# zengxiaofei/HapHiC

Hardware: NVIDIA H100
Metric: hic_pairs_per_sec_matrix_build (higher is better)
Workload: dtype int32 counts / fp32 matrix

## Files before the change

haphic_b200/csrc/hh_gemm.cu:

```cuda
#include "hh_common.cuh"
#include "hh_internal.cuh"
#include "hh_gemm.cuh"
#include <cuda.h>
#include <cuda_fp16.h>
#include <stdlib.h>
#include <algorithm>

__device__ __forceinline__ uint32_t hg_smem_u32(const void* p) { return (uint32_t)__cvta_generic_to_shared(p); }

__device__ __forceinline__ void hg_mbar_init(uint32_t bar, uint32_t count) {
    asm volatile("mbarrier.init.shared::cta.b64 [%0], %1;" ::"r"(bar), "r"(count) : "memory");
}
__device__ __forceinline__ void hg_fence_barrier_init() { asm volatile("fence.mbarrier_init.release.cluster;" ::: "memory"); }
__device__ __forceinline__ void hg_mbar_wait(uint32_t bar, uint32_t parity) {
    uint32_t ok;
    do {
        asm volatile(
            "{\n\t.reg .pred p;\n\t"
            "mbarrier.try_wait.parity.shared::cta.b64 p, [%1], %2;\n\t"
            "selp.u32 %0, 1, 0, p;\n\t}"
            : "=r"(ok)
            : "r"(bar), "r"(parity)
            : "memory");
    } while (!ok);
// ... 17 lines not shown
__device__ __forceinline__ uint64_t hg_make_desc(uint32_t saddr) {
    uint64_t d = 0;
    d |= (uint64_t)((saddr >> 4) & 0x3FFFu);
    d |= (uint64_t)1 << 16;
    d |= (uint64_t)(1024 >> 4) << 32;
    d |= (uint64_t)1 << 62;
    return d;
}

__device__ __forceinline__ void hg_wgmma_fence() { asm volatile("wgmma.fence.sync.aligned;" ::: "memory"); }
__device__ __forceinline__ void hg_wgmma_commit() { asm volatile("wgmma.commit_group.sync.aligned;" ::: "memory"); }
__device__ __forceinline__ void hg_wgmma_wait0() { asm volatile("wgmma.wait_group.sync.aligned 0;" ::: "memory"); }

#define HG_ACC8(i) "+f"(d[i]), "+f"(d[i + 1]), "+f"(d[i + 2]), "+f"(d[i + 3]), "+f"(d[i + 4]), "+f"(d[i + 5]), "+f"(d[i + 6]), "+f"(d[i + 7])
#define HG_WGMMA_BODY(TYPES)                                                                                                      \
    asm volatile(                                                                                                                 \
        "{\n\t.reg .pred p;\n\tsetp.ne.b32 p, %66, 0;\n\t"                                                                         \
        "wgmma.mma_async.sync.aligned.m64n128k16.f32." TYPES " "                                                                  \
        "{%0, %1, %2, %3, %4, %5, %6, %7, %8, %9, %10, %11, %12, %13, %14, %15, "                                                 \
        "%16, %17, %18, %19, %20, %21, %22, %23, %24, %25, %26, %27, %28, %29, %30, %31, "                                        \
        "%32, %33, %34, %35, %36, %37, %38, %39, %40, %41, %42, %43, %44, %45, %46, %47, "                                         \
        "%48, %49, %50, %51, %52, %53, %54, %55, %56, %57, %58, %59, %60, %61, %62, %63}, "                                       \
        "%64, %65, p, 1, 1, 0, 0;\n\t}"                                                                                           \
        : HG_ACC8(0), HG_ACC8(8), HG_ACC8(16), HG_ACC8(24), HG_ACC8(32), HG_ACC8(40), HG_ACC8(48), HG_ACC8(56)                   \
        : "l"(adesc), "l"(bdesc), "r"(accumulate))
template <bool F16>
__device__ __forceinline__ void hg_wgmma(float (&d)[64], uint64_t adesc, uint64_t bdesc, uint32_t accumulate) {
    if (F16) HG_WGMMA_BODY("f16.f16");
    else HG_WGMMA_BODY("bf16.bf16");
}

#define HG_THREADS 384
#define HG_TILE 128
#define HG_PLANE_BYTES 16384
#define HG_MAX_STAGES 4

struct hh_gemm_args {
    const hh_gemm_item* items;
    int n_items;
    int n;
    int na, nb;
    int npass;
    int pa[8], pb[8];
    int chunk_kb;
    int stages;
    float* m1;
    long long ld;
    int col_lo, col_hi;
    const float* inv_s;
    float out_scale;
    int accumulate;
};

template <bool F16>
__global__ void __launch_bounds__(HG_THREADS, 1)
hh_k_syrk(const __grid_constant__ CUtensorMap tmA, const __grid_constant__ CUtensorMap tmB, const hh_gemm_args a) {
    extern __shared__ uint8_t hg_smem_raw[];
    __shared__ __align__(8) uint64_t s_full[HG_MAX_STAGES];
    __shared__ __align__(8) uint64_t s_empty[HG_MAX_STAGES];

    const int wg = threadIdx.x >> 7, lane = threadIdx.x & 31;
    const uint32_t smem_base = (hg_smem_u32(hg_smem_raw) + 1023u) & ~1023u;
    const uint32_t stage_bytes = (uint32_t)(a.na + a.nb) * HG_PLANE_BYTES;
    const int S = a.stages;

    if (threadIdx.x == 0) {
        for (int s = 0; s < S; ++s) {
            hg_mbar_init(hg_smem_u32(&s_full[s]), 1);
            hg_mbar_init(hg_smem_u32(&s_empty[s]), 8);
        }
        hg_fence_barrier_init();
        hg_prefetch_tmap(&tmA);
        hg_prefetch_tmap(&tmB);
    }
    __syncthreads();

    if (wg == 0) {
        if (threadIdx.x == 0) {
            int s = 0;
            uint32_t ph = 0;
            for (int it = blockIdx.x; it < a.n_items; it += gridDim.x) {
                const hh_gemm_item w = a.items[it];
                for (int seg = 0; seg < 2; ++seg) {
                    for (int kb = w.kb_lo[seg]; kb < w.kb_hi[seg]; ++kb) {
                        hg_mbar_wait(hg_smem_u32(&s_empty[s]), ph ^ 1u);
                        const uint32_t bar = hg_smem_u32(&s_full[s]);
                        hg_mbar_expect_tx(bar, stage_bytes);
                        const uint32_t dst = smem_base + (uint32_t)s * stage_bytes;
                        for (int p = 0; p < a.na; ++p) hg_tma_load_3d(dst + (uint32_t)p * HG_PLANE_BYTES, &tmA, bar, kb * 64, w.m0, p);
                        for (int p = 0; p < a.nb; ++p)
                            hg_tma_load_3d(dst + (uint32_t)(a.na + p) * HG_PLANE_BYTES, &tmB, bar, kb * 64, w.n0, p);
                        if (++s == S) {
                            s = 0;
                            ph ^= 1u;
                        }
                    }
                }
            }
        }
        return;
    }

    const int e = wg - 1;
    const int wq = (threadIdx.x >> 5) & 3;
    int s = 0;
    uint32_t ph = 0;
    float acc[64], racc[64];
    for (int it = blockIdx.x; it < a.n_items; it += gridDim.x) {
        const hh_gemm_item w = a.items[it];
        const int total = (w.kb_hi[0] - w.kb_lo[0]) + (w.kb_hi[1] - w.kb_lo[1]);
#pragma unroll
        for (int j = 0; j < 64; ++j) {
            acc[j] = 0.f;
            racc[j] = 0.f;
        }
        int in_chunk = 0;
        for (int t = 0; t < total; ++t) {
            hg_mbar_wait(hg_smem_u32(&s_full[s]), ph);
            const uint32_t st = smem_base + (uint32_t)s * stage_bytes;
            hg_wgmma_fence();
            for (int p = 0; p < a.npass; ++p) {
                const uint64_t ad = hg_make_desc(st + (uint32_t)a.pa[p] * HG_PLANE_BYTES + (uint32_t)e * (64u * 128u));
                const uint64_t bd = hg_make_desc(st + (uint32_t)(a.na + a.pb[p]) * HG_PLANE_BYTES);
#pragma unroll
                for (int k = 0; k < 4; ++k)
                    hg_wgmma<F16>(acc, ad + (uint64_t)(2 * k), bd + (uint64_t)(2 * k), (in_chunk | p | k) ? 1u : 0u);
            }
            hg_wgmma_commit();
            hg_wgmma_wait0();
            __syncwarp();
            if (lane == 0) hg_mbar_arrive(hg_smem_u32(&s_empty[s]));
            if (++s == S) {
                s = 0;
                ph ^= 1u;
            }
            if (++in_chunk == a.chunk_kb || t + 1 == total) {
#pragma unroll
                for (int j = 0; j < 64; ++j) racc[j] = __fadd_rn(racc[j], acc[j]);
                in_chunk = 0;
            }
        }
#pragma unroll
        for (int h = 0; h < 2; ++h) {
            const int r = w.m0 + 64 * e + 16 * wq + (lane >> 2) + 8 * h;
            if (r >= w.m_end) continue;
            if (w.flags & HH_GEMM_DIRECT) {
                float* __restrict__ dst = a.m1 + (ptrdiff_t)(r - w.out_row0);
#pragma unroll
                for (int q = 0; q < 16; ++q) {
#pragma unroll
                    for (int b = 0; b < 2; ++b) {
                        const int c = w.n0 + 8 * q + 2 * (lane & 3) + b;
                        if (c < w.n_end && c >= a.col_lo && c < a.col_hi) {
                            float* __restrict__ o = dst + (size_t)(c - a.col_lo) * (size_t)a.ld;
                            const float x = racc[4 * q + 2 * h + b];
                            const float v = a.inv_s ? x * __ldg(a.inv_s + c) : x * a.out_scale;
                            *o = a.accumulate ? __fadd_rn(*o, v) : v;
                        }
                    }
                }
            }
            if ((w.flags & HH_GEMM_MIRROR) && r >= a.col_lo && r < a.col_hi) {
                const float sr = a.inv_s ? __ldg(a.inv_s + r) : a.out_scale;
                float* __restrict__ dst = a.m1 + (size_t)(r - a.col_lo) * (size_t)a.ld - (ptrdiff_t)w.out_row0;
#pragma unroll
                for (int q = 0; q < 16; ++q) {
                    const int c = w.n0 + 8 * q + 2 * (lane & 3);
                    const float v0 = racc[4 * q + 2 * h] * sr, v1 = racc[4 * q + 2 * h + 1] * sr;
                    if (c + 1 < w.n_end && w.out_row0 == 0) {
                        float2 v = make_float2(v0, v1);
                        if (a.accumulate) {
                            const float2 old = *reinterpret_cast<const float2*>(dst + c);
                            v = make_float2(__fadd_rn(old.x, v.x), __fadd_rn(old.y, v.y));
                        }
                        *reinterpret_cast<float2*>(dst + c) = v;
                    } else {
                        if (c < w.n_end) dst[c] = a.accumulate ? __fadd_rn(dst[c], v0) : v0;
                        if (c + 1 < w.n_end) dst[c + 1] = a.accumulate ? __fadd_rn(dst[c + 1], v1) : v1;
                    }
                }
            }
        }
    }
}

__global__ void hh_k_gemm_colsum(const int64_t* __restrict__ colptr, const float* __restrict__ val, int n, double* __restrict__ s,
                                 float* __restrict__ inv_s, int* __restrict__ flags) {
    const int c = blockIdx.x * (blockDim.x >> 5) + (threadIdx.x >> 5);
    if (c >= n) return;
    const int lane = threadIdx.x & 31;
    double t = 0.0;
    for (int64_t p = colptr[c] + lane; p < colptr[c + 1]; p += 32) t += fabs((double)val[p]);
    t = hh_warp_sum(t);
    if (lane == 0) {
        s[c] = t;
        inv_s[c] = (t != 0.0) ? (float)(1.0 / t) : 1.f;
        if (t >= 8388608.0) atomicOr(flags, 4);
    }
}

__global__ void hh_k_gemm_valstats(const float* __restrict__ val, int64_t nnz, int* __restrict__ flags) {
    int f = 0;
    for (int64_t p = (int64_t)blockIdx.x * blockDim.x + threadIdx.x; p < nnz; p += (int64_t)gridDim.x * blockDim.x) {
        const float v = val[p];
        if (!(v >= 0.f && v < 65536.f && v == floorf(v))) f |= 1;
        if (v > 256.f) f |= 2;
        if (v > 2048.f) f |= 8;
    }
    f = __reduce_or_sync(HH_FULL_MASK, f);
    if ((threadIdx.x & 31) == 0 && f) atomicOr(flags, f);
}

__device__ __forceinline__ void hg_split3(float x, unsigned short& h1, unsigned short& h2, unsigned short& h3) {
    const uint32_t b1 = __float_as_uint(x) & 0xFFFF0000u;
    const float r1 = x - __uint_as_float(b1);
// ... 13 lines not shown
    const int c = blockIdx.x;
    const int64_t p0 = colptr[c], p1 = colptr[c + 1];
    for (int group = 0; group < 2; ++group) {
        const int np = group ? nb : na;
        unsigned short* __restrict__ out = (group ? B : A) + (size_t)c * (size_t)ldk;
        for (long long seg0 = k0; seg0 < k0 + ldk; seg0 += HG_SEG) {
            const int seg_n = (int)((k0 + ldk - seg0 < HG_SEG) ? (k0 + ldk - seg0) : HG_SEG);
            uint4* z = reinterpret_cast<uint4*>(hg_row);
            for (int q = threadIdx.x; q < 3 * HG_SEG / 8; q += blockDim.x) z[q] = make_uint4(0u, 0u, 0u, 0u);
            __syncthreads();
            for (int64_t p = p0 + threadIdx.x; p < p1; p += blockDim.x) {
                const long long k = row[p];
                if (k < seg0 || k >= seg0 + seg_n) continue;
                const float v = fminf(val[p], clip);
                const double sk = s[k];
                unsigned short h1 = 0, h2 = 0, h3 = 0;
                if (!scaled) {
                    float x = v;
                    if (group) x = (sk != 0.0) ? (float)((double)v / sk) : v;
                    hg_split3(x, h1, h2, h3);
                } else {
                    const int e = (sk != 0.0) ? (int)((__double2hiint(sk) >> 20) & 0x7ff) - 1022 : 0;
                    if (!group) {
                        const float xa = v * __int_as_float((127 - e) << 23);
                        h1 = a_f16 ? __half_as_ushort(__float2half_rn(xa)) : (unsigned short)(__float_as_uint(xa) >> 16);
                    } else {
                        const float x = (sk != 0.0) ? (float)((double)v / sk) : v;
                        const float xs = x * __int_as_float((127 + e) << 23);
                        const __half hi = __float2half_rn(xs);
                        const __half lo = __float2half_rn(xs - __half2float(hi));
                        h1 = __half_as_ushort(hi);
                        h2 = __half_as_ushort(lo);
                    }
                }
                const int kk = (int)(k - seg0);
                hg_row[kk] = h1;
                if (np > 1) hg_row[HG_SEG + kk] = h2;
                if (np > 2) hg_row[2 * HG_SEG + kk] = h3;
            }
            __syncthreads();
            for (int pl = 0; pl < np; ++pl) {
                const uint4* src = reinterpret_cast<const uint4*>(hg_row + (size_t)pl * HG_SEG);
                uint4* dst = reinterpret_cast<uint4*>(out + (size_t)pl * (size_t)plane + (size_t)(seg0 - k0));
                for (int q = threadIdx.x; q < seg_n / 8; q += blockDim.x) dst[q] = src[q];
            }
            __syncthreads();
        }
    }
}

typedef CUresult (*hg_encode_fn)(CUtensorMap*, CUtensorMapDataType, cuuint32_t, void*, const cuuint64_t*, const cuuint64_t*, const cuuint32_t*,
                                 const cuuint32_t*, CUtensorMapInterleave, CUtensorMapSwizzle, CUtensorMapL2promotion, CUtensorMapFloatOOBfill);

static int hg_encode(CUtensorMap* tm, void* base, int rows, int kdim, long long ldk, long long plane_elems, int planes, int fmt) {
    static hg_encode_fn fn = nullptr;
    if (!fn) {
        void* p = nullptr;
        cudaDriverEntryPointQueryResult q;
        HH_CUDA(cudaGetDriverEntryPoint("cuTensorMapEncodeTiled", &p, cudaEnableDefault, &q));
        HH_REQUIRE(p != nullptr && q == cudaDriverEntryPointSuccess, HH_ERR_CUDA, "hh_gemm: the driver does not export cuTensorMapEncodeTiled");
        fn = reinterpret_cast<hg_encode_fn>(p);
    }
    const cuuint64_t dims[3] = {(cuuint64_t)kdim, (cuuint64_t)rows, (cuuint64_t)planes};
    const cuuint64_t strides[2] = {(cuuint64_t)ldk * 2ull, (cuuint64_t)plane_elems * 2ull};
    const cuuint32_t box[3] = {64u, 128u, 1u};
    const cuuint32_t estr[3] = {1u, 1u, 1u};
    const CUresult r = fn(tm, fmt == HH_GEMM_F16 ? CU_TENSOR_MAP_DATA_TYPE_FLOAT16 : CU_TENSOR_MAP_DATA_TYPE_BFLOAT16, 3, base, dims, strides, box, estr, CU_TENSOR_MAP_INTERLEAVE_NONE,
                          CU_TENSOR_MAP_SWIZZLE_128B, CU_TENSOR_MAP_L2_PROMOTION_L2_256B, CU_TENSOR_MAP_FLOAT_OOB_FILL_NONE);
    HH_REQUIRE(r == CUDA_SUCCESS, HH_ERR_CUDA, "hh_gemm: cuTensorMapEncodeTiled failed (%d)", (int)r);
    return HH_OK;
}

static int hg_env_int(const char* name, int dflt) {
    const char* v = getenv(name);
    return (v && *v) ? atoi(v) : dflt;
}

template <bool F16>
static int hg_launch(hh_ctx* ctx, const CUtensorMap& tmA, const CUtensorMap& tmB, const hh_gemm_args& a, size_t smem) {
    auto kern = hh_k_syrk<F16>;
    HH_CUDA(cudaFuncSetAttribute(kern, cudaFuncAttributeMaxDynamicSharedMemorySize, (int)smem));
    int grid = ctx->sm_count;
    if (grid > a.n_items) grid = a.n_items;
    if (grid < 1) grid = 1;
    HH_LAUNCH(ctx, kern, grid, HG_THREADS, smem, tmA, tmB, a);
    return HH_OK;
}

int hh_gemm_run(hh_ctx* ctx, const hh_gemm_operand& A, const hh_gemm_operand& B, const hh_gemm_item* d_items, int n_items, int npass,
                const int* pa, const int* pb, int chunk_kb, float* out, long long ld, int col_lo, int col_hi, const float* scale,
                int* stages_out, float out_scale, int accumulate) {
    HH_REQUIRE(n_items >= 1 && npass >= 1 && npass <= 8, HH_ERR_ARG, "hh_gemm_run: bad work list");
    HH_REQUIRE(A.fmt == B.fmt, HH_ERR_ARG, "hh_gemm_run: wgmma takes one 16-bit format for both operands");
    CUtensorMap tmA, tmB;
    HH_CHECK(hg_encode(&tmA, (void*)A.base, A.rows, A.kdim, A.ldk, A.plane, A.planes, A.fmt));
    HH_CHECK(hg_encode(&tmB, (void*)B.base, B.rows, B.kdim, B.ldk, B.plane, B.planes, B.fmt));
    hh_gemm_args a;
    memset(&a, 0, sizeof(a));
    a.items = d_items;
    a.n_items = n_items;
    a.na = A.planes;
    a.nb = B.planes;
    a.npass = npass;
    for (int p = 0; p < npass; ++p) {
        a.pa[p] = pa[p];
        a.pb[p] = pb[p];
    }
    a.chunk_kb = chunk_kb < 1 ? (1 << 30) : chunk_kb;
    const size_t stage_bytes = (size_t)(A.planes + B.planes) * HG_PLANE_BYTES;
    int stages = (int)((ctx->smem_optin - 2048) / stage_bytes);
    if (stages > HG_MAX_STAGES) stages = HG_MAX_STAGES;
    HH_REQUIRE(stages >= 2, HH_ERR_UNSUPPORTED, "hh_gemm: shared memory too small for two pipeline stages");
    a.stages = stages;
    if (stages_out) *stages_out = stages;
    a.m1 = out;
    a.ld = ld;
    a.col_lo = col_lo;
    a.col_hi = col_hi;
    a.inv_s = scale;
    a.out_scale = out_scale;
    a.accumulate = accumulate;
    const size_t smem = (size_t)stages * stage_bytes + 1024;
    return A.fmt == HH_GEMM_F16 ? hg_launch<true>(ctx, tmA, tmB, a, smem) : hg_launch<false>(ctx, tmA, tmB, a, smem);
}

static const int HG_P1[3][2] = {{0, 0}, {0, 1}, {0, 2}};
static const int HG_P3[6][2] = {{0, 0}, {0, 1}, {1, 0}, {0, 2}, {1, 1}, {2, 0}};

int hh_gemm_passes(int na, int* pa, int* pb) {
    const int(*pl)[2] = na == 1 ? HG_P1 : HG_P3;
    const int np = na == 1 ? 3 : 6;
    for (int p = 0; p < np; ++p) {
        pa[p] = pl[p][0];
        pb[p] = pl[p][1];
    }
    return np;
}

void hh_gemm_kchunks(int n, int planes, long long* kw_out, int* kchunks_out) {
    const long long ldk = ((long long)n + 63) & ~63ll;
    const double plane_bytes_all = (double)planes * (double)(ldk * (long long)n) * 2.0;
    int kchunks = (int)(plane_bytes_all / 16.0e9) + 1;
    kchunks = hg_env_int("HH_GEMM_KCHUNKS", kchunks);
    if (kchunks < 1) kchunks = 1;
    const long long kw = ((((long long)n + kchunks - 1) / kchunks) + 63) & ~63ll;
    *kw_out = kw;
    *kchunks_out = (int)(((long long)n + kw - 1) / kw);
}

size_t hh_gemm_preexpand_plane_bytes(int n) {
    size_t most = 0;
    for (int planes : {3, 4, 6}) {
        long long kw = 0;
        int kc = 0;
        hh_gemm_kchunks(n, planes, &kw, &kc);
        const size_t b = (size_t)planes * (size_t)kw * (size_t)n * 2;
        if (b > most) most = b;
    }
    return most;
}

int hh_gemm_preexpand(hh_ctx* ctx, const hh_matrix* m, int col_lo, int col_hi, float* d_m1, long long ld, const hh_gemm_item* h_items,
                      int n_items, hh_gemm_stats* st) {
    const int n = m->n;
    HH_REQUIRE(n >= 1 && n_items >= 1, HH_ERR_ARG, "hh_gemm_preexpand: empty problem");
    double* d_s = nullptr;
    float* d_inv = nullptr;
    int* d_flags = nullptr;
    unsigned short *d_A = nullptr, *d_B = nullptr;
    hh_gemm_item* d_items = nullptr;
    cudaEvent_t ev[3] = {nullptr, nullptr, nullptr};
    int rc = [&]() -> int {
        for (int k = 0; k < 3; ++k) HH_CUDA(cudaEventCreate(&ev[k]));
        HH_CHECK(hh_dmalloc(&d_s, (size_t)n));
        HH_CHECK(hh_dmalloc(&d_inv, (size_t)n));
        HH_CHECK(hh_dmalloc(&d_flags, 1));
        HH_CUDA(cudaEventRecord(ev[0], ctx->stream));
        HH_CUDA(cudaMemsetAsync(d_flags, 0, sizeof(int), ctx->stream));
        HH_LAUNCH(ctx, hh_k_gemm_colsum, (n + 7) / 8, 256, 0, m->d_colptr, m->d_val, n, d_s, d_inv, d_flags);
        HH_LAUNCH(ctx, hh_k_gemm_valstats, ctx->sm_count * 8, 256, 0, m->d_val, m->nnz, d_flags);
        int flags = 0;
        HH_CUDA(cudaMemcpyAsync(&flags, d_flags, sizeof(int), cudaMemcpyDeviceToHost, ctx->stream));
        HH_CUDA(cudaStreamSynchronize(ctx->stream));
        const char* fmt_env = getenv("HH_GEMM_FMT");
        int enc = 2;
        if (fmt_env && !strcmp(fmt_env, "bf16")) enc = 0;
        if (flags & (1 | 4)) enc = 0;
        const int na = (flags & 1) ? 3 : 1;
        const int nb = enc ? 2 : 3;
        const float clip = (flags & 1) ? 3.0e38f : (enc == 2 ? 2048.f : 256.f);
        const int fmt_a = enc == 2 ? HH_GEMM_F16 : HH_GEMM_BF16, fmt_b = enc ? HH_GEMM_F16 : HH_GEMM_BF16;
        long long kw = 0;
        int kchunks = 0;
        hh_gemm_kchunks(n, na + nb, &kw, &kchunks);
        const long long plane_c = kw * (long long)n;
        HH_CHECK(hh_ws_alloc(ctx, &d_A, (size_t)plane_c * (size_t)na));
        HH_CHECK(hh_ws_alloc(ctx, &d_B, (size_t)plane_c * (size_t)nb));
        HH_CUDA(cudaMemsetAsync(d_m1, 0, (size_t)ld * (size_t)(col_hi - col_lo) * sizeof(float), ctx->stream));
        HH_CHECK(hh_dmalloc(&d_items, (size_t)n_items));
        int pa[8], pb[8];
        int npass = hh_gemm_passes(na, pa, pb);
        if (enc) {
            npass = 2;
            pa[0] = pa[1] = 0;
            pb[0] = 0;
            pb[1] = 1;
        }
        const int chunk = hg_env_int("HH_GEMM_CHUNK", npass > 3 ? 1 : (npass == 3 ? 2 : 3));
        int stages = 0;
        float densify_ms = 0.f, gemm_ms = 0.f;
        const float stats_ms = 0.f;
        std::vector<hh_gemm_item> items_c(h_items, h_items + n_items);
        for (int kc = 0; kc < kchunks; ++kc) {
            const long long k0 = (long long)kc * kw;
            const long long k1 = std::min((long long)n, k0 + kw);
            HH_CUDA(cudaEventRecord(ev[0], ctx->stream));
            {
                auto kd = hh_k_gemm_densify;
                const size_t dsm = (size_t)3 * HG_SEG * sizeof(unsigned short);
                HH_CUDA(cudaFuncSetAttribute(kd, cudaFuncAttributeMaxDynamicSharedMemorySize, (int)dsm));
                HH_LAUNCH(ctx, kd, n, 1024, dsm, m->d_colptr, m->d_row, m->d_val, n, d_s, d_A, na, d_B, nb, kw, plane_c, clip, enc ? 1 : 0,
                          enc == 2 ? 1 : 0, k0);
            }
            const int nkb_c = (int)((k1 - k0 + 63) / 64);
            for (auto& w : items_c) {
                w.kb_lo[0] = 0;
                w.kb_hi[0] = nkb_c;
            }
            HH_CUDA(cudaMemcpyAsync(d_items, items_c.data(), (size_t)n_items * sizeof(hh_gemm_item), cudaMemcpyHostToDevice, ctx->stream));
            hh_gemm_operand A = {d_A, na, n, (int)(k1 - k0), kw, plane_c, fmt_a};
            hh_gemm_operand B = {d_B, nb, n, (int)(k1 - k0), kw, plane_c, fmt_b};
            HH_CUDA(cudaEventRecord(ev[1], ctx->stream));
            HH_CHECK(hh_gemm_run(ctx, A, B, d_items, n_items, npass, pa, pb, chunk, d_m1, ld, col_lo, col_hi, d_inv, &stages, 1.0f,
                                 kc > 0 ? 1 : 0));
            HH_CUDA(cudaEventRecord(ev[2], ctx->stream));
            HH_CUDA(cudaStreamSynchronize(ctx->stream));
            float t0 = 0.f, t1 = 0.f;
            HH_CUDA(cudaEventElapsedTime(&t0, ev[0], ev[1]));
            HH_CUDA(cudaEventElapsedTime(&t1, ev[1], ev[2]));
            densify_ms += t0;
            gemm_ms += t1;
        }
        HH_CUDA(cudaEventRecord(ev[2], ctx->stream));
        HH_CUDA(cudaStreamSynchronize(ctx->stream));
        if (st) {
            memset(st, 0, sizeof(*st));
            st->a_planes = na;
            st->clipped = (clip < 1.0e38f && (flags & (clip > 256.f ? 8 : 2))) ? 1 : 0;
            st->clip = clip;
            st->fmt_a = fmt_a;
            st->fmt_b = fmt_b;
            st->b_planes = nb;
            st->passes = npass;
            st->cta_group = 1;
            st->stages = stages;
            st->chunk_kb = chunk < 1 ? (1 << 30) : chunk;
            st->densify_ms = densify_ms + stats_ms;
            st->gemm_ms = gemm_ms;
            st->k_chunks = kchunks;
            double kb = 0.0;
            for (int i = 0; i < n_items; ++i) kb += (double)((h_items[i].kb_hi[0] - h_items[i].kb_lo[0]) + (h_items[i].kb_hi[1] - h_items[i].kb_lo[1]));
            const double tile = (double)HG_TILE;
            st->flops = 2.0 * tile * tile * 64.0 * kb * (double)npass;
        }
        return HH_OK;
    }();
    hh_dfree(d_s);
    hh_dfree(d_inv);
    hh_dfree(d_flags);
    hh_ws_free(ctx, d_A);
    hh_ws_free(ctx, d_B);
    hh_dfree(d_items);
    for (int k = 0; k < 3; ++k)
        if (ev[k]) cudaEventDestroy(ev[k]);
    return rc;
}


#define HG_BLK_SHIFT 14
__global__ void __launch_bounds__(128)
hh_k_blk_densify(const int* __restrict__ len, const uint2* __restrict__ ent, int cap, const int* __restrict__ list, int nlist,
                 const int* __restrict__ comp_lo, const int* __restrict__ comp_hi, unsigned short* __restrict__ Bt, long long ldk,
                 long long plane, int f16) {
    extern __shared__ __align__(16) unsigned short hb_row[];
    const int j = list[blockIdx.x];
    const int lo = comp_lo[j], width = comp_hi[j] - lo;
    uint4* z = reinterpret_cast<uint4*>(hb_row);
    for (int q = threadIdx.x; q < (int)(3 * ldk / 8); q += 128) z[q] = make_uint4(0u, 0u, 0u, 0u);
    __syncthreads();
    const int L = len[j];
    const uint2* __restrict__ e = ent + (size_t)j * (size_t)cap;
    for (int p = threadIdx.x; p < L; p += 128) {
        const uint2 t = e[p];
        const unsigned kk = t.x - (unsigned)lo;
        if (kk < (unsigned)width) {
            unsigned short h1, h2, h3 = 0;
            if (f16) {
                const float xs = ldexpf(__uint_as_float(t.y), HG_BLK_SHIFT);
                const __half hi = __float2half_rn(xs);
                h1 = __half_as_ushort(hi);
                h2 = __half_as_ushort(__float2half_rn(xs - __half2float(hi)));
            } else {
                hg_split3(__uint_as_float(t.y), h1, h2, h3);
            }
            hb_row[kk] = h1;
            hb_row[ldk + kk] = h2;
            hb_row[2 * ldk + kk] = h3;
        }
    }
    __syncthreads();
    for (int pl = 0; pl < (f16 ? 2 : 3); ++pl) {
        const uint4* src = reinterpret_cast<const uint4*>(hb_row + (size_t)pl * (size_t)ldk);
        uint4* dst = reinterpret_cast<uint4*>(Bt + (size_t)pl * (size_t)plane + (size_t)j * (size_t)ldk);
        for (int q = threadIdx.x; q < (int)(ldk / 8); q += 128) dst[q] = src[q];
    }
}

__global__ void __launch_bounds__(256)
hh_k_blk_transpose(const unsigned short* __restrict__ Bt, unsigned short* __restrict__ A, int n, const int* __restrict__ comp_lo,
                   const int* __restrict__ comp_hi, long long ldk, long long plane) {
    __shared__ unsigned short tile[32][34];
    const int r0 = blockIdx.x * 32, kk0 = blockIdx.y * 32;
    const unsigned short* __restrict__ src = Bt + (size_t)blockIdx.z * (size_t)plane;
    unsigned short* __restrict__ dst = A + (size_t)blockIdx.z * (size_t)plane;
    const int tx = threadIdx.x, ty = threadIdx.y;
    const int rl = min(r0 + 31, n - 1);
    const bool same = (r0 + 31 < n) && comp_lo[r0] == comp_lo[rl];
    if (same) {
        const int lo = comp_lo[r0], width = comp_hi[r0] - lo;
        const bool fits = width <= (int)ldk;
        for (int y = ty; y < 32; y += 8) {
            const int kk = kk0 + y;
            tile[y][tx] = (fits && kk < width) ? src[(size_t)(lo + kk) * (size_t)ldk + (size_t)(r0 - lo + tx)] : (unsigned short)0;
        }
        __syncthreads();
        for (int y = ty; y < 32; y += 8) dst[(size_t)(r0 + y) * (size_t)ldk + (size_t)(kk0 + tx)] = tile[tx][y];
    } else {
        for (int y = ty; y < 32; y += 8) {
            const int r = r0 + y;
            if (r >= n) continue;
            const int lo = comp_lo[r], width = comp_hi[r] - lo;
            const int kk = kk0 + tx;
            dst[(size_t)r * (size_t)ldk + (size_t)kk] =
                (width <= (int)ldk && kk < width) ? src[(size_t)(lo + kk) * (size_t)ldk + (size_t)(r - lo)] : (unsigned short)0;
        }
    }
}

float hh_gemm_blk_out_scale(int f16) { return f16 ? ldexpf(1.0f, -2 * HG_BLK_SHIFT) : 1.0f; }

int hh_gemm_blk_operands(hh_ctx* ctx, const int* d_len, const void* d_ent, int cap, const int* d_list, int nlist, const int* d_comp_lo,
                         const int* d_comp_hi, int n, unsigned short* d_A, unsigned short* d_Bt, long long ldk, int f16) {
    const long long plane = ldk * (long long)n;
    auto kd = hh_k_blk_densify;
    const size_t dsm = (size_t)3 * (size_t)ldk * sizeof(unsigned short);
    HH_CUDA(cudaFuncSetAttribute(kd, cudaFuncAttributeMaxDynamicSharedMemorySize, (int)dsm));
    if (nlist > 0)
        HH_LAUNCH(ctx, kd, nlist, 128, dsm, d_len, reinterpret_cast<const uint2*>(d_ent), cap, d_list, nlist, d_comp_lo, d_comp_hi, d_Bt, ldk,
                  plane, f16);
    dim3 grid((unsigned)((n + 31) / 32), (unsigned)(ldk / 32), f16 ? 2u : 3u), block(32, 8);
    hh_k_blk_transpose<<<grid, block, 0, ctx->stream>>>(d_Bt, d_A, n, d_comp_lo, d_comp_hi, ldk, plane);
    ctx->launches++;
    HH_CUDA(cudaGetLastError());
    return HH_OK;
}

int hh_gemm_tile_size() { return HG_TILE; }

int hh_gemm_items_full(int n, int col_lo, int col_hi, std::vector<hh_gemm_item>& out) {
    const int T = hh_gemm_tile_size();
    const int nt = (n + T - 1) / T;
    const int nkb = (n + 63) / 64;
    out.clear();
    auto owned = [&](int t) {
        const int c0 = t * T, c1 = std::min(n, c0 + T);
        return c1 > col_lo && c0 < col_hi;
    };
    const int SB_M = 16, SB_N = 8;
    for (int bb = 0; bb < nt; bb += SB_N) {
        for (int ba = 0; ba <= std::min(nt - 1, bb + SB_N - 1); ba += SB_M) {
            for (int ta = ba; ta < std::min(nt, ba + SB_M); ++ta) {
                for (int tb = std::max(bb, ta); tb < std::min(nt, bb + SB_N); ++tb) {
                    int flags = 0;
                    if (owned(tb)) flags |= HH_GEMM_DIRECT;
                    if (tb > ta && owned(ta)) flags |= HH_GEMM_MIRROR;
                    if (!flags) continue;
                    hh_gemm_item w;
                    memset(&w, 0, sizeof(w));
                    w.m0 = ta * T;
                    w.n0 = tb * T;
                    w.m_end = n;
                    w.n_end = n;
                    w.kb_lo[0] = 0;
                    w.kb_hi[0] = nkb;
                    w.flags = flags;
                    out.push_back(w);
                }
            }
        }
    }
    return HH_OK;
}
```

haphic_b200/csrc/hh_gemm.cuh:

```cuda
#pragma once
#include "hh_common.cuh"
#include "hh_internal.cuh"
#include <vector>

enum { HH_GEMM_DIRECT = 1, HH_GEMM_MIRROR = 2 };

struct hh_gemm_item {
    int m0, n0;
    int m_end, n_end;
    int kb_lo[2], kb_hi[2];
    int flags;
    int out_row0;
    int pad[2];
};

enum { HH_GEMM_BF16 = 0, HH_GEMM_F16 = 1 };
struct hh_gemm_operand {
    const unsigned short* base;
    int planes;
    int rows, kdim;
    long long ldk, plane;
    int fmt;
};

struct hh_gemm_stats {
    int a_planes, passes, cta_group, stages, chunk_kb;
    int clipped;
    float clip;
    int fmt_a, fmt_b;
    int b_planes;
    int k_chunks;
    float densify_ms, gemm_ms;
    double flops;
};

int hh_gemm_tile_size();
int hh_gemm_items_full(int n, int col_lo, int col_hi, std::vector<hh_gemm_item>& out);
int hh_gemm_preexpand(hh_ctx* ctx, const hh_matrix* m, int col_lo, int col_hi, float* d_m1, long long ld, const hh_gemm_item* h_items,
                      int n_items, hh_gemm_stats* st);
int hh_gemm_run(hh_ctx* ctx, const hh_gemm_operand& A, const hh_gemm_operand& B, const hh_gemm_item* d_items, int n_items, int npass,
                const int* pa, const int* pb, int chunk_kb, float* out, long long ld, int col_lo, int col_hi, const float* scale,
                int* stages_out, float out_scale, int accumulate);
int hh_gemm_passes(int na, int* pa, int* pb);
void hh_gemm_kchunks(int n, int planes, long long* kw, int* kchunks);
size_t hh_gemm_preexpand_plane_bytes(int n);

int hh_gemm_blk_operands(hh_ctx* ctx, const int* d_len, const void* d_ent, int cap, const int* d_list, int nlist, const int* d_comp_lo,
                         const int* d_comp_hi, int n, unsigned short* d_A, unsigned short* d_Bt, long long ldk, int f16);
float hh_gemm_blk_out_scale(int f16);
```

haphic_b200/csrc/hh_mcl.cu:

```cuda
#include "hh_common.cuh"
#include "hh_internal.cuh"
#include "hh_gemm.cuh"
#include <math.h>
#include <stdlib.h>
#include <algorithm>
#include <utility>

struct hh_slotmat {
    int n;
    int cap;
    int W;
    int* len;
    int* blk;
    uint2* ent;
};

enum { HH_INFL_POW = 0, HH_INFL_SQUARE = 1, HH_INFL_X15 = 2, HH_INFL_CUBE = 3, HH_INFL_X25 = 4 };
__device__ __forceinline__ float hh_inflate(float x, float rf, int mode) {
    switch (mode) {
        case HH_INFL_SQUARE: return x * x;
        case HH_INFL_X15: return x * __fsqrt_rn(x);
        case HH_INFL_CUBE: return (x * x) * x;
        case HH_INFL_X25: return (x * x) * __fsqrt_rn(x);
        default: return powf(x, rf);
// ... 2064 lines not shown
    mc->own_hi = col_hi;
    mc->expansion = expansion;
    mc->cur = -1;
    mc->use_blk = (expansion == 2) ? env_int("HH_MCL_BLOCKGEMM", 1) : 0;
    mc->info.it = -1;
    mc->blk_items = new std::vector<hh_gemm_item>();
    const hh_geom g = geom_for(ctx, m->n);
    mc->W = g.W;
    mc->T = g.T;
    mc->ch_shift = g.ch_shift;
    mc->n_pad = g.n_pad;
    mc->smem_acc = g.smem_acc;
    mc->smem_bytes = g.smem_bytes;
    mc->ld = ((int64_t)m->n + 31) & ~31ll;
    int rc = [&]() -> int {
        HH_CHECK(grid_cap_for(ctx, g, &mc->grid_cap));
        HH_CUDA(cudaEventCreate(&mc->ev0));
        HH_CUDA(cudaEventCreate(&mc->ev1));
        if (!g.smem_acc) HH_CHECK(hh_dmalloc(&mc->d_scratch, (size_t)mc->grid_cap * (size_t)g.n_pad));
        HH_CHECK(hh_dmalloc(&mc->d_counter, 1));
        HH_CHECK(hh_dmalloc(&mc->d_stats, 4));
        HH_CHECK(hh_dmalloc(&mc->d_order, (size_t)m->n));
        HH_CHECK(hh_dmalloc(&mc->d_cnt, (size_t)m->n * 2));
        HH_CHECK(hh_dmalloc(&mc->d_bigcount, 4));
        HH_CHECK(hh_dmalloc(&mc->d_perm, (size_t)m->n));
        HH_CHECK(hh_dmalloc(&mc->d_inv, (size_t)m->n));
        HH_CHECK(hh_dmalloc(&mc->d_comp_lo, (size_t)m->n));
        HH_CHECK(hh_dmalloc(&mc->d_comp_hi, (size_t)m->n));
        HH_CHECK(hh_dmalloc(&mc->d_owned, (size_t)m->n));
        HH_CHECK(hh_dmalloc(&mc->d_win_list, (size_t)m->n));
        HH_CHECK(hh_dmalloc(&mc->d_big_list, (size_t)m->n));
        HH_CHECK(hh_dmalloc(&mc->d_overflow, (size_t)m->n));
        HH_CUDA(cudaMemsetAsync(mc->d_stats, 0, 4 * sizeof(unsigned long long), ctx->stream));
        int cap0 = 0;
        HH_CHECK(max_col_len(ctx, m, &cap0));
        HH_CHECK(slot_alloc(mc->m0, m->n, cap0, g.W));
        HH_CUDA(cudaEventRecord(mc->ev0, ctx->stream));
        HH_CHECK(slot_from_csc(ctx, g, mc->d_scratch, mc->grid_cap, mc->d_counter, mc->d_stats, m, 0, mc->m0));
        HH_CUDA(cudaEventRecord(mc->ev1, ctx->stream));
        unsigned long long st[4];
        HH_CHECK(read_stats(ctx, mc->d_stats, st));
        HH_CUDA(cudaEventElapsedTime(&mc->create_ms[0], mc->ev0, mc->ev1));
        HH_REQUIRE((int)st[3] == 0, HH_ERR_CAPACITY, "hh_mcl_create: column slot overflow while normalising");
        mc->nnz_m0 = (int64_t)st[0];
        const int ncols = col_hi - col_lo;
        HH_CHECK(hh_dmalloc(&mc->d_m1, (size_t)mc->ld * (size_t)ncols));
        HH_CUDA(cudaMemsetAsync(mc->d_stats, 0, 4 * sizeof(unsigned long long), ctx->stream));
        mc->preexp_mode = (expansion == 2) ? choose_preexp(m, preexp_mode) : HH_PREEXP_SPARSE;
        if (expansion > 2) {
            HH_CHECK(slot_alloc(mc->pw[0], m->n, m->n, g.W));
            if (expansion > 3) HH_CHECK(slot_alloc(mc->pw[1], m->n, m->n, g.W));
        }
        if (mc->preexp_mode == HH_PREEXP_DENSE) {
            std::vector<hh_gemm_item> items;
            HH_CHECK(hh_gemm_items_full(m->n, col_lo, col_hi, items));
            HH_CHECK(hh_gemm_preexpand(ctx, m, col_lo, col_hi, mc->d_m1, mc->ld, items.data(), (int)items.size(), &mc->gemm));
            mc->create_ms[1] = mc->gemm.densify_ms + mc->gemm.gemm_ms;
            mc->preexp_products = 0;
            if (mc->gemm.clipped) {
                float* d_bclip = nullptr;
                double* d_s = nullptr;
                int rc2 = [&]() -> int {
                    HH_CHECK(hh_dmalloc(&d_bclip, (size_t)m->n));
                    HH_CHECK(hh_dmalloc(&d_s, (size_t)m->n));
                    HH_CUDA(cudaMemsetAsync(mc->d_stats, 0, 4 * sizeof(unsigned long long), ctx->stream));
                    HH_CUDA(cudaEventRecord(mc->ev0, ctx->stream));
                    const int grid = (m->n + 7) / 8;
                    HH_LAUNCH(ctx, hh_k_clip_stats, grid, 256, 0, m->d_colptr, m->d_val, m->n, d_s, d_bclip, mc->gemm.clip);
                    HH_LAUNCH(ctx, hh_k_clip_fix<0>, grid, 256, 0, mc->m0, d_s, d_bclip, mc->d_m1, (long long)mc->ld, (int)col_lo, (int)col_hi,
                              mc->d_stats + 1, mc->gemm.clip);
                    HH_LAUNCH(ctx, hh_k_clip_fix<1>, grid, 256, 0, mc->m0, d_s, d_bclip, mc->d_m1, (long long)mc->ld, (int)col_lo, (int)col_hi,
                              mc->d_stats + 1, mc->gemm.clip);
                    HH_CUDA(cudaEventRecord(mc->ev1, ctx->stream));
                    unsigned long long st2[4];
                    HH_CHECK(read_stats(ctx, mc->d_stats, st2));
                    float ms = 0.f;
                    HH_CUDA(cudaEventElapsedTime(&ms, mc->ev0, mc->ev1));
                    mc->clip_ms = ms;
                    mc->create_ms[1] += ms;
                    mc->preexp_products = (int64_t)st2[1];
                    return HH_OK;
                }();
                hh_dfree(d_bclip);
                hh_dfree(d_s);
                HH_CHECK(rc2);
            }
            return HH_OK;
        }
        const hh_slotmat* Bp = &mc->m0;
        HH_CUDA(cudaEventRecord(mc->ev0, ctx->stream));
        for (int pwr = 2; pwr < expansion; ++pwr) {
            HH_CHECK(raw_product(mc, mc->m0, *Bp, (double)mc->nnz_m0, mc->pw[pwr & 1]));
            Bp = &mc->pw[pwr & 1];
        }
        if (expansion > 2) {
            HH_CHECK(read_stats(ctx, mc->d_stats, st));
            HH_REQUIRE((int)(st[3] & 0xffffffffull) == 0, HH_ERR_CAPACITY, "hh_mcl_create: slot overflow in a matrix power");
        }
        hh_colargs a;
        mcl_base_args(mc, a);
        a.A = mc->m0;
        a.B = *Bp;
        a.dense_out = mc->d_m1;
        a.flat = choose_flat(mc, (double)mc->nnz_m0);
        const int n = m->n;
        int* d_lab = mc->d_comp_lo;
        int* d_flag = mc->d_bigcount + 2;
        HH_LAUNCH(ctx, hh_k_cc_init, (n + 255) / 256, 256, 0, d_lab, n);
        int gridc = (n + 7) / 8;
// ... 581 lines not shown
```

Before: 6.220 billion.

## Use 192-row GEMM tiles with three consumer warpgroups and an inline producer

Adds a variant of the SYRK wgmma kernel whose A tile is 192 rows. It is processed by three consumer warpgroups, and thread 0 of the first consumer issues the TMA loads inline instead of a dedicated producer warpgroup. Work items are regenerated for 192-row panels with per-64-row slice flags so direct and mirror writes stay correct across the triangular tiles. This is meant to raise the ratio of B-tile reuse to loaded bytes and drop the idle producer warpgroup. In exchange, the larger stage means fewer pipeline stages, and some tiles near the diagonal do extra work. It is the default when the plane count is small, and HH_GEMM_ROWS can override it.

```diff
diff --git a/haphic_b200/csrc/hh_gemm.cu b/haphic_b200/csrc/hh_gemm.cu
--- a/haphic_b200/csrc/hh_gemm.cu
+++ b/haphic_b200/csrc/hh_gemm.cu
@@ -93,22 +93,58 @@
     int accumulate;
 };
 
-template <bool F16>
+struct hg_feed {
+    int it, seg, kb, s;
+    uint32_t ph;
+};
+
+template <int W>
+__device__ __forceinline__ bool hg_feed_next(hg_feed& f, const hh_gemm_args& a, const CUtensorMap* tmA, const CUtensorMap* tmB,
+                                             uint32_t smem_base, uint32_t stage_bytes, uint32_t full0, uint32_t empty0) {
+    constexpr uint32_t a_plane = (uint32_t)W * 64u * 128u;
+    while (f.it < a.n_items && f.kb >= a.items[f.it].kb_hi[f.seg]) {
+        if (++f.seg == 2) {
+            f.seg = 0;
+            f.it += gridDim.x;
+        }
+        if (f.it < a.n_items) f.kb = a.items[f.it].kb_lo[f.seg];
+    }
+    if (f.it >= a.n_items) return false;
+    const int m0 = a.items[f.it].m0, n0 = a.items[f.it].n0;
+    hg_mbar_wait(empty0 + 8u * (uint32_t)f.s, f.ph ^ 1u);
+    const uint32_t bar = full0 + 8u * (uint32_t)f.s;
+    hg_mbar_expect_tx(bar, stage_bytes);
+    const uint32_t dst = smem_base + (uint32_t)f.s * stage_bytes;
+    for (int p = 0; p < a.na; ++p) hg_tma_load_3d(dst + (uint32_t)p * a_plane, tmA, bar, f.kb * 64, m0, p);
+    for (int p = 0; p < a.nb; ++p) hg_tma_load_3d(dst + (uint32_t)a.na * a_plane + (uint32_t)p * HG_PLANE_BYTES, tmB, bar, f.kb * 64, n0, p);
+    ++f.kb;
+    if (++f.s == a.stages) {
+        f.s = 0;
+        f.ph ^= 1u;
+    }
+    return true;
+}
+
+template <bool F16, int W>
 __global__ void __launch_bounds__(HG_THREADS, 1)
 hh_k_syrk(const __grid_constant__ CUtensorMap tmA, const __grid_constant__ CUtensorMap tmB, const hh_gemm_args a) {
+    static_assert(W == 2 || W == 3, "two consumer warpgroups and a producer, or three consumers");
+    constexpr int kFirst = W == 2 ? 1 : 0;
+    constexpr uint32_t a_plane = (uint32_t)W * 64u * 128u;
     extern __shared__ uint8_t hg_smem_raw[];
     __shared__ __align__(8) uint64_t s_full[HG_MAX_STAGES];
     __shared__ __align__(8) uint64_t s_empty[HG_MAX_STAGES];
 
     const int wg = threadIdx.x >> 7, lane = threadIdx.x & 31;
     const uint32_t smem_base = (hg_smem_u32(hg_smem_raw) + 1023u) & ~1023u;
-    const uint32_t stage_bytes = (uint32_t)(a.na + a.nb) * HG_PLANE_BYTES;
+    const uint32_t stage_bytes = (uint32_t)a.na * a_plane + (uint32_t)a.nb * HG_PLANE_BYTES;
+    const uint32_t full0 = hg_smem_u32(&s_full[0]), empty0 = hg_smem_u32(&s_empty[0]);
     const int S = a.stages;
 
     if (threadIdx.x == 0) {
         for (int s = 0; s < S; ++s) {
-            hg_mbar_init(hg_smem_u32(&s_full[s]), 1);
-            hg_mbar_init(hg_smem_u32(&s_empty[s]), 8);
+            hg_mbar_init(full0 + 8u * (uint32_t)s, 1);
+            hg_mbar_init(empty0 + 8u * (uint32_t)s, 4 * W);
         }
         hg_fence_barrier_init();
         hg_prefetch_tmap(&tmA);
@@ -116,61 +152,50 @@
     }
     __syncthreads();
 
-    if (wg == 0) {
-        if (threadIdx.x == 0) {
-            int s = 0;
-            uint32_t ph = 0;
-            for (int it = blockIdx.x; it < a.n_items; it += gridDim.x) {
-                const hh_gemm_item w = a.items[it];
-                for (int seg = 0; seg < 2; ++seg) {
-                    for (int kb = w.kb_lo[seg]; kb < w.kb_hi[seg]; ++kb) {
-                        hg_mbar_wait(hg_smem_u32(&s_empty[s]), ph ^ 1u);
-                        const uint32_t bar = hg_smem_u32(&s_full[s]);
-                        hg_mbar_expect_tx(bar, stage_bytes);
-                        const uint32_t dst = smem_base + (uint32_t)s * stage_bytes;
-                        for (int p = 0; p < a.na; ++p) hg_tma_load_3d(dst + (uint32_t)p * HG_PLANE_BYTES, &tmA, bar, kb * 64, w.m0, p);
-                        for (int p = 0; p < a.nb; ++p)
-                            hg_tma_load_3d(dst + (uint32_t)(a.na + p) * HG_PLANE_BYTES, &tmB, bar, kb * 64, w.n0, p);
-                        if (++s == S) {
-                            s = 0;
-                            ph ^= 1u;
-                        }
-                    }
-                }
-            }
-        }
+    hg_feed feed = {(int)blockIdx.x, 0, blockIdx.x < (unsigned)a.n_items ? a.items[blockIdx.x].kb_lo[0] : 0, 0, 0u};
+    if (W == 2 && wg == 0) {
+        if (threadIdx.x == 0)
+            while (hg_feed_next<W>(feed, a, &tmA, &tmB, smem_base, stage_bytes, full0, empty0)) {}
         return;
     }
-
-    const int e = wg - 1;
+    if (W == 3 && threadIdx.x == 0)
+        for (int s = 0; s < S && hg_feed_next<W>(feed, a, &tmA, &tmB, smem_base, stage_bytes, full0, empty0); ++s) {}
+
+    const int e = wg - kFirst;
     const int wq = (threadIdx.x >> 5) & 3;
     int s = 0;
     uint32_t ph = 0;
+    int step = 0;
     float acc[64], racc[64];
     for (int it = blockIdx.x; it < a.n_items; it += gridDim.x) {
         const hh_gemm_item w = a.items[it];
         const int total = (w.kb_hi[0] - w.kb_lo[0]) + (w.kb_hi[1] - w.kb_lo[1]);
+        const int flags = W == 2 ? w.flags : (w.slice_flags >> (2 * e)) & 3;
 #pragma unroll
         for (int j = 0; j < 64; ++j) {
             acc[j] = 0.f;
             racc[j] = 0.f;
         }
         int in_chunk = 0;
-        for (int t = 0; t < total; ++t) {
-            hg_mbar_wait(hg_smem_u32(&s_full[s]), ph);
+        for (int t = 0; t < total; ++t, ++step) {
+            hg_mbar_wait(full0 + 8u * (uint32_t)s, ph);
             const uint32_t st = smem_base + (uint32_t)s * stage_bytes;
-            hg_wgmma_fence();
-            for (int p = 0; p < a.npass; ++p) {
-                const uint64_t ad = hg_make_desc(st + (uint32_t)a.pa[p] * HG_PLANE_BYTES + (uint32_t)e * (64u * 128u));
-                const uint64_t bd = hg_make_desc(st + (uint32_t)(a.na + a.pb[p]) * HG_PLANE_BYTES);
+            {
+                hg_wgmma_fence();
+                for (int p = 0; p < a.npass; ++p) {
+                    const uint64_t ad = hg_make_desc(st + (uint32_t)a.pa[p] * a_plane + (uint32_t)e * (64u * 128u));
+                    const uint64_t bd = hg_make_desc(st + (uint32_t)a.na * a_plane + (uint32_t)a.pb[p] * HG_PLANE_BYTES);
 #pragma unroll
-                for (int k = 0; k < 4; ++k)
-                    hg_wgmma<F16>(acc, ad + (uint64_t)(2 * k), bd + (uint64_t)(2 * k), (in_chunk | p | k) ? 1u : 0u);
-            }
-            hg_wgmma_commit();
+                    for (int k = 0; k < 4; ++k)
+                        hg_wgmma<F16>(acc, ad + (uint64_t)(2 * k), bd + (uint64_t)(2 * k), (in_chunk | p | k) ? 1u : 0u);
+                }
+                hg_wgmma_commit();
+            }
+            if (W == 3 && threadIdx.x == 0 && step > 0) hg_feed_next<W>(feed, a, &tmA, &tmB, smem_base, stage_bytes, full0, empty0);
+            __syncwarp();
             hg_wgmma_wait0();
             __syncwarp();
-            if (lane == 0) hg_mbar_arrive(hg_smem_u32(&s_empty[s]));
+            if (lane == 0) hg_mbar_arrive(empty0 + 8u * (uint32_t)s);
             if (++s == S) {
                 s = 0;
                 ph ^= 1u;
@@ -185,7 +210,7 @@
         for (int h = 0; h < 2; ++h) {
             const int r = w.m0 + 64 * e + 16 * wq + (lane >> 2) + 8 * h;
             if (r >= w.m_end) continue;
-            if (w.flags & HH_GEMM_DIRECT) {
+            if (flags & HH_GEMM_DIRECT) {
                 float* __restrict__ dst = a.m1 + (ptrdiff_t)(r - w.out_row0);
 #pragma unroll
                 for (int q = 0; q < 16; ++q) {
@@ -201,7 +226,7 @@
                     }
                 }
             }
-            if ((w.flags & HH_GEMM_MIRROR) && r >= a.col_lo && r < a.col_hi) {
+            if ((flags & HH_GEMM_MIRROR) && r >= a.col_lo && r < a.col_hi) {
                 const float sr = a.inv_s ? __ldg(a.inv_s + r) : a.out_scale;
                 float* __restrict__ dst = a.m1 + (size_t)(r - a.col_lo) * (size_t)a.ld - (ptrdiff_t)w.out_row0;
 #pragma unroll
@@ -321,7 +346,8 @@
 typedef CUresult (*hg_encode_fn)(CUtensorMap*, CUtensorMapDataType, cuuint32_t, void*, const cuuint64_t*, const cuuint64_t*, const cuuint32_t*,
                                  const cuuint32_t*, CUtensorMapInterleave, CUtensorMapSwizzle, CUtensorMapL2promotion, CUtensorMapFloatOOBfill);
 
-static int hg_encode(CUtensorMap* tm, void* base, int rows, int kdim, long long ldk, long long plane_elems, int planes, int fmt) {
+static int hg_encode(CUtensorMap* tm, void* base, int rows, int kdim, long long ldk, long long plane_elems, int planes, int fmt,
+                     int box_rows) {
     static hg_encode_fn fn = nullptr;
     if (!fn) {
         void* p = nullptr;
@@ -332,7 +358,7 @@
     }
     const cuuint64_t dims[3] = {(cuuint64_t)kdim, (cuuint64_t)rows, (cuuint64_t)planes};
     const cuuint64_t strides[2] = {(cuuint64_t)ldk * 2ull, (cuuint64_t)plane_elems * 2ull};
-    const cuuint32_t box[3] = {64u, 128u, 1u};
+    const cuuint32_t box[3] = {64u, (cuuint32_t)box_rows, 1u};
     const cuuint32_t estr[3] = {1u, 1u, 1u};
     const CUresult r = fn(tm, fmt == HH_GEMM_F16 ? CU_TENSOR_MAP_DATA_TYPE_FLOAT16 : CU_TENSOR_MAP_DATA_TYPE_BFLOAT16, 3, base, dims, strides, box, estr, CU_TENSOR_MAP_INTERLEAVE_NONE,
                           CU_TENSOR_MAP_SWIZZLE_128B, CU_TENSOR_MAP_L2_PROMOTION_L2_256B, CU_TENSOR_MAP_FLOAT_OOB_FILL_NONE);
@@ -345,9 +371,9 @@
     return (v && *v) ? atoi(v) : dflt;
 }
 
-template <bool F16>
+template <bool F16, int W>
 static int hg_launch(hh_ctx* ctx, const CUtensorMap& tmA, const CUtensorMap& tmB, const hh_gemm_args& a, size_t smem) {
-    auto kern = hh_k_syrk<F16>;
+    auto kern = hh_k_syrk<F16, W>;
     HH_CUDA(cudaFuncSetAttribute(kern, cudaFuncAttributeMaxDynamicSharedMemorySize, (int)smem));
     int grid = ctx->sm_count;
     if (grid > a.n_items) grid = a.n_items;
@@ -358,12 +384,13 @@
 
 int hh_gemm_run(hh_ctx* ctx, const hh_gemm_operand& A, const hh_gemm_operand& B, const hh_gemm_item* d_items, int n_items, int npass,
                 const int* pa, const int* pb, int chunk_kb, float* out, long long ld, int col_lo, int col_hi, const float* scale,
-                int* stages_out, float out_scale, int accumulate) {
+                int* stages_out, float out_scale, int accumulate, int rows) {
     HH_REQUIRE(n_items >= 1 && npass >= 1 && npass <= 8, HH_ERR_ARG, "hh_gemm_run: bad work list");
     HH_REQUIRE(A.fmt == B.fmt, HH_ERR_ARG, "hh_gemm_run: wgmma takes one 16-bit format for both operands");
+    HH_REQUIRE(rows == 128 || rows == 192, HH_ERR_ARG, "hh_gemm_run: items of %d rows (128 or 192)", rows);
     CUtensorMap tmA, tmB;
-    HH_CHECK(hg_encode(&tmA, (void*)A.base, A.rows, A.kdim, A.ldk, A.plane, A.planes, A.fmt));
-    HH_CHECK(hg_encode(&tmB, (void*)B.base, B.rows, B.kdim, B.ldk, B.plane, B.planes, B.fmt));
+    HH_CHECK(hg_encode(&tmA, (void*)A.base, A.rows, A.kdim, A.ldk, A.plane, A.planes, A.fmt, rows));
+    HH_CHECK(hg_encode(&tmB, (void*)B.base, B.rows, B.kdim, B.ldk, B.plane, B.planes, B.fmt, HG_TILE));
     hh_gemm_args a;
     memset(&a, 0, sizeof(a));
     a.items = d_items;
@@ -376,7 +403,7 @@
         a.pb[p] = pb[p];
     }
     a.chunk_kb = chunk_kb < 1 ? (1 << 30) : chunk_kb;
-    const size_t stage_bytes = (size_t)(A.planes + B.planes) * HG_PLANE_BYTES;
+    const size_t stage_bytes = (size_t)A.planes * (size_t)(rows * 128) + (size_t)B.planes * HG_PLANE_BYTES;
     int stages = (int)((ctx->smem_optin - 2048) / stage_bytes);
     if (stages > HG_MAX_STAGES) stages = HG_MAX_STAGES;
     HH_REQUIRE(stages >= 2, HH_ERR_UNSUPPORTED, "hh_gemm: shared memory too small for two pipeline stages");
@@ -390,7 +417,8 @@
     a.out_scale = out_scale;
     a.accumulate = accumulate;
     const size_t smem = (size_t)stages * stage_bytes + 1024;
-    return A.fmt == HH_GEMM_F16 ? hg_launch<true>(ctx, tmA, tmB, a, smem) : hg_launch<false>(ctx, tmA, tmB, a, smem);
+    if (rows == 192) return A.fmt == HH_GEMM_F16 ? hg_launch<true, 3>(ctx, tmA, tmB, a, smem) : hg_launch<false, 3>(ctx, tmA, tmB, a, smem);
+    return A.fmt == HH_GEMM_F16 ? hg_launch<true, 2>(ctx, tmA, tmB, a, smem) : hg_launch<false, 2>(ctx, tmA, tmB, a, smem);
 }
 
 static const int HG_P1[3][2] = {{0, 0}, {0, 1}, {0, 2}};
@@ -429,10 +457,9 @@
     return most;
 }
 
-int hh_gemm_preexpand(hh_ctx* ctx, const hh_matrix* m, int col_lo, int col_hi, float* d_m1, long long ld, const hh_gemm_item* h_items,
-                      int n_items, hh_gemm_stats* st) {
+int hh_gemm_preexpand(hh_ctx* ctx, const hh_matrix* m, int col_lo, int col_hi, float* d_m1, long long ld, hh_gemm_stats* st) {
     const int n = m->n;
-    HH_REQUIRE(n >= 1 && n_items >= 1, HH_ERR_ARG, "hh_gemm_preexpand: empty problem");
+    HH_REQUIRE(n >= 1, HH_ERR_ARG, "hh_gemm_preexpand: empty problem");
     double* d_s = nullptr;
     float* d_inv = nullptr;
     int* d_flags = nullptr;
@@ -466,6 +493,11 @@
         HH_CHECK(hh_ws_alloc(ctx, &d_A, (size_t)plane_c * (size_t)na));
         HH_CHECK(hh_ws_alloc(ctx, &d_B, (size_t)plane_c * (size_t)nb));
         HH_CUDA(cudaMemsetAsync(d_m1, 0, (size_t)ld * (size_t)(col_hi - col_lo) * sizeof(float), ctx->stream));
+        const int rows = (na + nb <= 4) ? hg_env_int("HH_GEMM_ROWS", 192) : 128;
+        HH_REQUIRE(rows == 128 || rows == 192, HH_ERR_ARG, "hh_gemm_preexpand: HH_GEMM_ROWS must be 128 or 192, not %d", rows);
+        std::vector<hh_gemm_item> items_c;
+        HH_CHECK(hh_gemm_items_full(n, col_lo, col_hi, rows, items_c));
+        const int n_items = (int)items_c.size();
         HH_CHECK(hh_dmalloc(&d_items, (size_t)n_items));
         int pa[8], pb[8];
         int npass = hh_gemm_passes(na, pa, pb);
@@ -479,7 +511,6 @@
         int stages = 0;
         float densify_ms = 0.f, gemm_ms = 0.f;
         const float stats_ms = 0.f;
-        std::vector<hh_gemm_item> items_c(h_items, h_items + n_items);
         for (int kc = 0; kc < kchunks; ++kc) {
             const long long k0 = (long long)kc * kw;
             const long long k1 = std::min((long long)n, k0 + kw);
@@ -501,7 +532,7 @@
             hh_gemm_operand B = {d_B, nb, n, (int)(k1 - k0), kw, plane_c, fmt_b};
             HH_CUDA(cudaEventRecord(ev[1], ctx->stream));
             HH_CHECK(hh_gemm_run(ctx, A, B, d_items, n_items, npass, pa, pb, chunk, d_m1, ld, col_lo, col_hi, d_inv, &stages, 1.0f,
-                                 kc > 0 ? 1 : 0));
+                                 kc > 0 ? 1 : 0, rows));
             HH_CUDA(cudaEventRecord(ev[2], ctx->stream));
             HH_CUDA(cudaStreamSynchronize(ctx->stream));
             float t0 = 0.f, t1 = 0.f;
@@ -527,10 +558,8 @@
             st->densify_ms = densify_ms + stats_ms;
             st->gemm_ms = gemm_ms;
             st->k_chunks = kchunks;
-            double kb = 0.0;
-            for (int i = 0; i < n_items; ++i) kb += (double)((h_items[i].kb_hi[0] - h_items[i].kb_lo[0]) + (h_items[i].kb_hi[1] - h_items[i].kb_lo[1]));
-            const double tile = (double)HG_TILE;
-            st->flops = 2.0 * tile * tile * 64.0 * kb * (double)npass;
+            const double nkb = (double)((n + 63) / 64);
+            st->flops = 2.0 * (double)rows * (double)HG_TILE * 64.0 * nkb * (double)n_items * (double)npass;
         }
         return HH_OK;
     }();
@@ -636,33 +665,40 @@
 
 int hh_gemm_tile_size() { return HG_TILE; }
 
-int hh_gemm_items_full(int n, int col_lo, int col_hi, std::vector<hh_gemm_item>& out) {
+int hh_gemm_items_full(int n, int col_lo, int col_hi, int rows, std::vector<hh_gemm_item>& out) {
     const int T = hh_gemm_tile_size();
     const int nt = (n + T - 1) / T;
+    const int np = (n + rows - 1) / rows;
     const int nkb = (n + 63) / 64;
     out.clear();
-    auto owned = [&](int t) {
-        const int c0 = t * T, c1 = std::min(n, c0 + T);
-        return c1 > col_lo && c0 < col_hi;
-    };
-    const int SB_M = 16, SB_N = 8;
+    auto owned = [&](int r0, int r1) { return std::min(n, r1) > col_lo && r0 < col_hi; };
+    const int SB_M = rows == 128 ? 16 : 11, SB_N = rows == 128 ? 8 : 12;
     for (int bb = 0; bb < nt; bb += SB_N) {
-        for (int ba = 0; ba <= std::min(nt - 1, bb + SB_N - 1); ba += SB_M) {
-            for (int ta = ba; ta < std::min(nt, ba + SB_M); ++ta) {
-                for (int tb = std::max(bb, ta); tb < std::min(nt, bb + SB_N); ++tb) {
-                    int flags = 0;
-                    if (owned(tb)) flags |= HH_GEMM_DIRECT;
-                    if (tb > ta && owned(ta)) flags |= HH_GEMM_MIRROR;
+        const int tb_end = std::min(nt, bb + SB_N);
+        for (int ba = 0; ba < np && ba * rows / T < tb_end; ba += SB_M) {
+            for (int pm = ba; pm < std::min(np, ba + SB_M); ++pm) {
+                for (int tb = bb; tb < tb_end; ++tb) {
+                    int flags = 0, slice_flags = 0;
+                    for (int g = 0; g < rows / 64; ++g) {
+                        const int r0 = pm * rows + 64 * g, ta = r0 / T;
+                        if (r0 >= n || ta > tb) continue;
+                        int f = 0;
+                        if (owned(tb * T, tb * T + T)) f |= HH_GEMM_DIRECT;
+                        if (tb > ta && owned(r0, r0 + 64)) f |= HH_GEMM_MIRROR;
+                        flags |= f;
+                        slice_flags |= f << (2 * g);
+                    }
                     if (!flags) continue;
                     hh_gemm_item w;
                     memset(&w, 0, sizeof(w));
-                    w.m0 = ta * T;
+                    w.m0 = pm * rows;
                     w.n0 = tb * T;
                     w.m_end = n;
                     w.n_end = n;
                     w.kb_lo[0] = 0;
                     w.kb_hi[0] = nkb;
                     w.flags = flags;
+                    w.slice_flags = slice_flags;
                     out.push_back(w);
                 }
             }
diff --git a/haphic_b200/csrc/hh_gemm.cuh b/haphic_b200/csrc/hh_gemm.cuh
--- a/haphic_b200/csrc/hh_gemm.cuh
+++ b/haphic_b200/csrc/hh_gemm.cuh
@@ -11,7 +11,8 @@
     int kb_lo[2], kb_hi[2];
     int flags;
     int out_row0;
-    int pad[2];
+    int slice_flags;
+    int pad;
 };
 
 enum { HH_GEMM_BF16 = 0, HH_GEMM_F16 = 1 };
@@ -35,12 +36,11 @@
 };
 
 int hh_gemm_tile_size();
-int hh_gemm_items_full(int n, int col_lo, int col_hi, std::vector<hh_gemm_item>& out);
-int hh_gemm_preexpand(hh_ctx* ctx, const hh_matrix* m, int col_lo, int col_hi, float* d_m1, long long ld, const hh_gemm_item* h_items,
-                      int n_items, hh_gemm_stats* st);
+int hh_gemm_items_full(int n, int col_lo, int col_hi, int rows, std::vector<hh_gemm_item>& out);
+int hh_gemm_preexpand(hh_ctx* ctx, const hh_matrix* m, int col_lo, int col_hi, float* d_m1, long long ld, hh_gemm_stats* st);
 int hh_gemm_run(hh_ctx* ctx, const hh_gemm_operand& A, const hh_gemm_operand& B, const hh_gemm_item* d_items, int n_items, int npass,
                 const int* pa, const int* pb, int chunk_kb, float* out, long long ld, int col_lo, int col_hi, const float* scale,
-                int* stages_out, float out_scale, int accumulate);
+                int* stages_out, float out_scale, int accumulate, int rows = 128);
 int hh_gemm_passes(int na, int* pa, int* pb);
 void hh_gemm_kchunks(int n, int planes, long long* kw, int* kchunks);
 size_t hh_gemm_preexpand_plane_bytes(int n);
diff --git a/haphic_b200/csrc/hh_mcl.cu b/haphic_b200/csrc/hh_mcl.cu
--- a/haphic_b200/csrc/hh_mcl.cu
+++ b/haphic_b200/csrc/hh_mcl.cu
@@ -2140,9 +2140,7 @@
             if (expansion > 3) HH_CHECK(slot_alloc(mc->pw[1], m->n, m->n, g.W));
         }
         if (mc->preexp_mode == HH_PREEXP_DENSE) {
-            std::vector<hh_gemm_item> items;
-            HH_CHECK(hh_gemm_items_full(m->n, col_lo, col_hi, items));
-            HH_CHECK(hh_gemm_preexpand(ctx, m, col_lo, col_hi, mc->d_m1, mc->ld, items.data(), (int)items.size(), &mc->gemm));
+            HH_CHECK(hh_gemm_preexpand(ctx, m, col_lo, col_hi, mc->d_m1, mc->ld, &mc->gemm));
             mc->create_ms[1] = mc->gemm.densify_ms + mc->gemm.gemm_ms;
             mc->preexp_products = 0;
             if (mc->gemm.clipped) {
```

After: 6.245 billion (median of 6 runs). About the same (+0.4%).
